# lhoyer/improving_segmentation_with_selfsupervised_depth

Measured on AMD Instinct MI355X. Metric: train images/sec, ResNet-101 joint seg+depth @512x1024, higher is better.
Workload: dtype f32

## Files before the change

### improving_segmentation_with_selfsupervised_depth_amd/csrc/winograd_fused.hip

```cpp
#include <stdlib.h>
#include <type_traits>
#include "segsde_common.h"
#include "winograd.h"
#ifndef WINO_UP_SKIP
#define WINO_UP_SKIP 1
#endif

namespace {
#define ST(s) static_cast<hipStream_t>(s)
constexpr int FT_H = 4, FT_W = 8;
constexpr int FP_H = 2 * FT_H + 2, FP_W = 2 * FT_W + 2;
constexpr int FROW = 20, FODD = FP_W / 2;
constexpr int FPS = 256;
__device__ __forceinline__ constexpr int fplane(int c) { return c * FPS + 2 * (c >> 2); }
constexpr int FCH = 64;
constexpr int FZP = 36;
constexpr int F_FLOATS = 8 * 64 * FZP > FCH * FPS ? 8 * 64 * FZP : FCH * FPS;
#ifdef WINO_DBG_OCC1
constexpr size_t F_LDS = 96 * 1024;
#else
constexpr size_t F_LDS = (size_t)F_FLOATS * sizeof(float) + 2 * 4 * 64 * sizeof(double);
#endif

struct WinoSrc { const float* x0; const float* x1; int ld0, ld1, C0, up0; };
struct WinoAg { const float* agy; int agld, agkind; };

template <bool STATS, bool UBLK, bool UPSKIP>
__global__ __launch_bounds__(256, 2) void wino_fused_kernel(WinoSrc src, int B, int H, int W, int C, int reflect,
                                                            const float* U, int ldu, int Co, const float* bias, int act, float* y, int ldy,
                                                            double* part, int accumulate, WinoAg ag) {
  SEGSDE_SMEM;
  float* lds = reinterpret_cast<float*>(segsde_smem);
  double* sh = reinterpret_cast<double*>(lds + F_FLOATS);
  const int H2 = H >> 1, W2 = W >> 1;
  const int nbw = (W2 + FT_W - 1) / FT_W, nbh = (H2 + FT_H - 1) / FT_H;
  const int tid = threadIdx.x, lane = tid & 63, wave = tid >> 6;
  const int t = lane & 31, kk = lane >> 5, th = t >> 3, tw = t & 7;
  const int bidx = blockIdx.x;
  int blk = segsde_xcd_remap(bidx, gridDim.x);
  const int bw = blk % nbw; blk /= nbw;
  const int bh = blk % nbh; const int b = blk / nbh;
  const int co0 = blockIdx.y * 64;
  const int h_top = 2 * bh * FT_H - 1, w_left = 2 * bw * FT_W - 1;
  const int a1 = wave == 0 ? 0 : (wave == 2 ? 2 : 1);
  const int a2 = wave == 0 ? 2 : (wave == 1 ? 2 : (wave == 2 ? 1 : 3));
  const float sgn = wave == 1 ? 1.f : -1.f;
  const float* pl = lds + kk * FPS + (2 * th) * FROW + tw;
  const int o1 = a1 * FROW, o2 = a2 * FROW;

  f32x16 acc[4][2];
#pragma unroll
  for (int j = 0; j < 4; ++j)
#pragma unroll
    for (int nb = 0; nb < 2; ++nb)
#pragma unroll
      for (int r = 0; r < 16; ++r) acc[j][nb][r] = 0.f;

  constexpr int NL = (FP_H * FP_W * (FCH / 4) + 255) / 256;
  unsigned poff[NL];
  int cur_src = -1, lds_ = 0;
  long img = 0;
  int sh_ = 0, Ws = 0;
  auto patch_offset = [&](int i) -> unsigned {
    const int e = tid + 256 * i;
    const int pix = e >> 4, cq = e & 15;
    const int pr = pix / FP_W, pos = pix - pr * FP_W;
    const int pc = pos < FODD ? 2 * pos : 2 * (pos - FODD) + 1;
    int hh = h_top + pr, ww = w_left + pc;
    if (reflect) {
      hh = hh < 0 ? -hh : (hh >= H ? 2 * H - 2 - hh : hh); ww = ww < 0 ? -ww : (ww >= W ? 2 * W - 2 - ww : ww);
      hh = hh < 0 ? 0 : hh; ww = ww < 0 ? 0 : ww;
    }
    const bool ok = e < FP_H * FP_W * (FCH / 4) && (unsigned)hh < (unsigned)H && (unsigned)ww < (unsigned)W;
    return ok ? (unsigned)(((hh >> sh_) * Ws + (ww >> sh_)) * lds_ + 4 * cq) * 4u : SEGSDE_OOB;
  };

  for (int c0 = 0; c0 < C; c0 += FCH) {
#ifdef WINO_DBG_LOOP_ONLY
    if (c0 == 0)
#endif
    {
    __syncthreads();
    {
      float4 v[NL];
      const int sidx = c0 < src.C0 ? 0 : 1;
      const bool first = sidx != cur_src;
      if (first) {
        cur_src = sidx;
        sh_ = (sidx == 0 && src.up0) ? 1 : 0;
        Ws = W >> sh_;
        lds_ = sidx == 0 ? src.ld0 : src.ld1;
        img = (long)(H >> sh_) * Ws * lds_;
      }
      const float* xs = sidx == 0 ? src.x0 : src.x1;
      const segsde_rsrc xr = segsde_make_rsrc(xs + (size_t)b * img + (sidx == 0 ? c0 : c0 - src.C0));
#ifdef WINO_DBG_SKIP_LOAD
      (void)xr; (void)first;
#pragma unroll
      for (int i = 0; i < NL; ++i) { poff[i] = patch_offset(i); v[i] = make_float4((float)poff[i], 1.f, 2.f, 3.f); }
#else
      if (first) {
#pragma unroll
        for (int i = 0; i < NL; ++i) { poff[i] = patch_offset(i); v[i] = segsde_buffer_load4(xr, poff[i], 0u); }
      } else {
#pragma unroll
        for (int i = 0; i < NL; ++i) v[i] = segsde_buffer_load4(xr, poff[i], 0u);
      }
#endif
#pragma unroll
      for (int i = 0; i < NL; ++i) {
        const int e = tid + 256 * i;
        if (e < FP_H * FP_W * (FCH / 4)) {
          const int pix = e >> 4, pr = pix / FP_W;
          float* d = lds + fplane(4 * (e & 15)) + pr * FROW + (pix - pr * FP_W);
          d[0] = v[i].x; d[FPS] = v[i].y; d[2 * FPS] = v[i].z; d[3 * FPS] = v[i].w;
        }
      }
    }
    __syncthreads();
    }
    const int wave_u = __builtin_amdgcn_readfirstlane(wave);
    const segsde_rsrc ur = segsde_make_rsrc(U);
    const unsigned nb64 = (unsigned)(ldu >> 6);
    const unsigned lane_off = UBLK ? (unsigned)(kk * nb64 * 256 + t * 8) * 4u : (unsigned)(kk * ldu + t) * 4u;
    const unsigned ubase = UBLK ? (unsigned)((((long)wave_u * C + c0) * nb64 + (co0 >> 6)) * 256 * 4)
                                : (unsigned)((((long)(4 * wave_u) * C + c0) * ldu + co0) * 4);
    const unsigned upos = (unsigned)((long)C * ldu * 4), ustep = UBLK ? 2u * nb64 * 256u * 4u : (unsigned)(2 * ldu * 4);
    constexpr int PD = 4, NS = FCH / 2;
    float bv[PD][8], rv[2][8];
    auto fetch_b = [&](int s, int q) {
      const unsigned so = ubase + (unsigned)s * ustep;
      if constexpr (UBLK) {
        const float4 lo = segsde_buffer_load4(ur, lane_off, so), hi = segsde_buffer_load4(ur, lane_off, so + 16u);
        bv[q][0] = lo.x; bv[q][1] = lo.y; bv[q][2] = lo.z; bv[q][3] = lo.w;
        bv[q][4] = hi.x; bv[q][5] = hi.y; bv[q][6] = hi.z; bv[q][7] = hi.w;
      } else {
#pragma unroll
        for (int j = 0; j < 4; ++j) {
          bv[q][2 * j] = segsde_buffer_load1(ur, lane_off, so + j * upos);
          bv[q][2 * j + 1] = segsde_buffer_load1(ur, lane_off, so + j * upos + 128u);
        }
      }
    };
#ifdef WINO_DBG_SKIP_K
    constexpr int NS_RUN = 1;
#else
    constexpr int NS_RUN = NS;
#endif
    float An[2][4];
    auto form_a = [&](int q, int h) {
      if (h == 0) {
        const float e0 = __builtin_fmaf(rv[0][4], sgn, rv[0][0]), e1 = __builtin_fmaf(rv[0][5], sgn, rv[0][1]);
        const float e2 = __builtin_fmaf(rv[0][6], sgn, rv[0][2]);
        An[q][0] = e0 - e2; An[q][1] = e1 + e2; An[q][2] = e2 - e1; rv[1][0] = e1;
      } else {
        const float e3 = __builtin_fmaf(rv[0][7], sgn, rv[0][3]);
        An[q][3] = rv[1][0] - e3;
      }
    };
    auto fetch_a2 = [&](int s, int bb) {
      const float* src = pl + fplane(2 * s);
      const int cp = (bb & 1) ? FODD + (bb >> 1) : (bb >> 1);
      rv[0][bb] = SEGSDE_LDS_READ_IMM(src + o1, cp); rv[0][4 + bb] = SEGSDE_LDS_READ_IMM(src + o2, cp);
    };
    const bool skip2 = UPSKIP && c0 < src.C0;
    if (!(skip2 && wave_u == 2)) {
#pragma unroll
      for (int s = 0; s < PD - 1; ++s) fetch_b(s, s);
#pragma unroll
      for (int bb = 0; bb < 4; ++bb) fetch_a2(0, bb);
      form_a(0, 0); form_a(0, 1);
      __builtin_amdgcn_sched_barrier(0);
#pragma unroll
      for (int s = 0; s < NS_RUN; ++s) {
        const int q = s & 1, qb = s % PD;
        const bool nx = s + 1 < NS;
#define WINO_MF_(j, nb, bi) acc[j][nb] = __builtin_amdgcn_mfma_f32_32x32x2f32(An[q][j], bv[qb][bi], acc[j][nb], 0, 0, 0); __builtin_amdgcn_sched_barrier(0)
        WINO_MF_(0, 0, 0); if (nx) fetch_a2(s + 1, 0); __builtin_amdgcn_sched_barrier(0);
        WINO_MF_(0, 1, 1); if (nx) fetch_a2(s + 1, 1); __builtin_amdgcn_sched_barrier(0);
        WINO_MF_(1, 0, 2); if (nx) fetch_a2(s + 1, 2); __builtin_amdgcn_sched_barrier(0);
        WINO_MF_(1, 1, 3); if (nx) fetch_a2(s + 1, 3); __builtin_amdgcn_sched_barrier(0);
        if (!skip2) {
          WINO_MF_(2, 0, 4); __builtin_amdgcn_sched_barrier(0);
          WINO_MF_(2, 1, 5); __builtin_amdgcn_sched_barrier(0);
        }
        if (s + PD - 1 < NS) fetch_b(s + PD - 1, (s + PD - 1) % PD);
        __builtin_amdgcn_sched_barrier(0);
        WINO_MF_(3, 0, 6); if (nx) form_a(q ^ 1, 0); __builtin_amdgcn_sched_barrier(0);
        WINO_MF_(3, 1, 7); if (nx) form_a(q ^ 1, 1); __builtin_amdgcn_sched_barrier(0);
#undef WINO_MF_
      }
    }
  }

#ifdef WINO_DBG_SKIP_EPI
  {
    float sdbg = 0.f;
#pragma unroll
    for (int j = 0; j < 4; ++j)
#pragma unroll
      for (int nb = 0; nb < 2; ++nb)
#pragma unroll
        for (int r = 0; r < 16; ++r) sdbg += acc[j][nb][r];
    if (sdbg == 1.2345678f) y[0] = sdbg;
    return;
  }
#endif
  __syncthreads();
  {
    float* zw = lds + ((2 * wave) * 64 + t) * FZP + 4 * kk;
#pragma unroll
    for (int nb = 0; nb < 2; ++nb)
#pragma unroll
      for (int rg = 0; rg < 4; ++rg) {
        float4 c0v, c1v;
        float* a0 = reinterpret_cast<float*>(&c0v);
        float* a1 = reinterpret_cast<float*>(&c1v);
#pragma unroll
        for (int i = 0; i < 4; ++i) {
          const int r = 4 * rg + i;
          const float m0 = acc[0][nb][r], m1 = acc[1][nb][r], m2 = acc[2][nb][r], m3 = acc[3][nb][r];
          a0[i] = (m0 + m1) + m2;
          a1[i] = (m1 - m2) - m3;
        }
        *reinterpret_cast<float4*>(zw + (nb * 32) * FZP + 8 * rg) = c0v;
        *reinterpret_cast<float4*>(zw + (64 + nb * 32) * FZP + 8 * rg) = c1v;
      }
  }
  const int n = tid & 63, tg = __builtin_amdgcn_readfirstlane(tid >> 6);
  const bool post = bias != nullptr || act != SEGSDE_ACT_NONE;
  const int co = co0 + n;
  const int ti = bh * FT_H + tg;
  const unsigned lane_b = (unsigned)co * 4u;
#ifdef WINO_EPI_POINTERS
  constexpr bool kBuf = false;
#else
  constexpr bool kBuf = true;
#endif
  const segsde_rsrc yr = segsde_make_rsrc(y + (long)b * H * W * ldy);
  const segsde_rsrc agr = segsde_make_rsrc(ag.agy ? ag.agy + (long)b * H * W * ag.agld : y);
  float agv[FT_W][4], oldv[FT_W][4];
  if (ag.agy) {
#pragma unroll
    for (int q = 0; q < FT_W; ++q) {
      const int tj = bw * FT_W + q;
      const bool ok = ti < H2 && tj < W2;
      if (kBuf) {
        const unsigned s0 = (unsigned)((2 * ti) * W + 2 * tj) * (unsigned)ag.agld * 4u, sr = (unsigned)W * (unsigned)ag.agld * 4u;
        if (ok) {
          agv[q][0] = segsde_buffer_load1(agr, lane_b, s0); agv[q][1] = segsde_buffer_load1(agr, lane_b, s0 + (unsigned)ag.agld * 4u);
          agv[q][2] = segsde_buffer_load1(agr, lane_b, s0 + sr); agv[q][3] = segsde_buffer_load1(agr, lane_b, s0 + sr + (unsigned)ag.agld * 4u);
        } else { agv[q][0] = agv[q][1] = agv[q][2] = agv[q][3] = 0.f; }
      } else {
        const float* ap = ag.agy + ((long)(b * H + 2 * ti) * W + 2 * tj) * ag.agld + co;
        agv[q][0] = ok ? ap[0] : 0.f; agv[q][1] = ok ? ap[ag.agld] : 0.f;
        agv[q][2] = ok ? ap[(long)W * ag.agld] : 0.f; agv[q][3] = ok ? ap[(long)W * ag.agld + ag.agld] : 0.f;
      }
    }
  }
  if (accumulate & 1) {
#pragma unroll
    for (int q = 0; q < FT_W; ++q) {
      const int tj = bw * FT_W + q;
      const bool ok = ti < H2 && tj < W2;
      if (kBuf) {
        const unsigned s0 = (unsigned)((2 * ti) * W + 2 * tj) * (unsigned)ldy * 4u, sr = (unsigned)W * (unsigned)ldy * 4u;
        if (ok) {
          oldv[q][0] = segsde_buffer_load1(yr, lane_b, s0); oldv[q][1] = segsde_buffer_load1(yr, lane_b, s0 + (unsigned)ldy * 4u);
          oldv[q][2] = segsde_buffer_load1(yr, lane_b, s0 + sr); oldv[q][3] = segsde_buffer_load1(yr, lane_b, s0 + sr + (unsigned)ldy * 4u);
        } else { oldv[q][0] = oldv[q][1] = oldv[q][2] = oldv[q][3] = 0.f; }
      } else {
        const float* yp = y + ((long)(b * H + 2 * ti) * W + 2 * tj) * ldy + co;
        oldv[q][0] = ok ? yp[0] : 0.f; oldv[q][1] = ok ? yp[ldy] : 0.f;
        oldv[q][2] = ok ? yp[(long)W * ldy] : 0.f; oldv[q][3] = ok ? yp[(long)W * ldy + ldy] : 0.f;
      }
    }
  }
  __syncthreads();
  const float bsv = bias ? bias[co] : 0.f;
  double ssum = 0.0, ssq = 0.0;
  float zall[4][2][FT_W];
  {
    const float* zp = lds + n * FZP + tg * FT_W;
#pragma unroll
    for (int i = 0; i < 4; ++i)
#pragma unroll
      for (int c = 0; c < 2; ++c)
#pragma unroll
        for (int h = 0; h < FT_W / 4; ++h) {
          const float4 v = *reinterpret_cast<const float4*>(zp + ((2 * i + c) * 64) * FZP + 4 * h);
          zall[i][c][4 * h] = v.x; zall[i][c][4 * h + 1] = v.y; zall[i][c][4 * h + 2] = v.z; zall[i][c][4 * h + 3] = v.w;
        }
  }
#pragma unroll
  for (int q = 0; q < FT_W; ++q) {
    float z0[4], z1[4];
#pragma unroll
    for (int i = 0; i < 4; ++i) { z0[i] = zall[i][0][q]; z1[i] = zall[i][1][q]; }
    float o[4];
    o[0] = (z0[0] + z0[1]) + z0[2]; o[1] = (z1[0] + z1[1]) + z1[2];
    o[2] = (z0[1] - z0[2]) - z0[3]; o[3] = (z1[1] - z1[2]) - z1[3];
    if (post) {
#pragma unroll
      for (int k = 0; k < 4; ++k) o[k] = segsde_act(o[k] + bsv, act);
    }
    const int tj = bw * FT_W + q;
    if (ti < H2 && tj < W2) {
      float* yp = y + ((long)(b * H + 2 * ti) * W + 2 * tj) * ldy + co;
      if (ag.agy) {
#pragma unroll
        for (int k = 0; k < 4; ++k) o[k] *= segsde_act_grad_from_out(agv[q][k], ag.agkind);
      }
      if (accumulate & 1) {
#pragma unroll
        for (int k = 0; k < 4; ++k) o[k] += oldv[q][k];
      }
#ifdef WINO_DBG_FEW_STORES
      if (q == 0)
#endif
      if (kBuf) {
        const unsigned s0 = (unsigned)((2 * ti) * W + 2 * tj) * (unsigned)ldy * 4u, sr = (unsigned)W * (unsigned)ldy * 4u, sc = (unsigned)ldy * 4u;
        if (accumulate & 2) {
          segsde_buffer_store1_nt(yr, lane_b, s0, o[0]); segsde_buffer_store1_nt(yr, lane_b, s0 + sc, o[1]);
          segsde_buffer_store1_nt(yr, lane_b, s0 + sr, o[2]); segsde_buffer_store1_nt(yr, lane_b, s0 + sr + sc, o[3]);
        } else {
          segsde_buffer_store1(yr, lane_b, s0, o[0]); segsde_buffer_store1(yr, lane_b, s0 + sc, o[1]);
          segsde_buffer_store1(yr, lane_b, s0 + sr, o[2]); segsde_buffer_store1(yr, lane_b, s0 + sr + sc, o[3]);
        }
      } else if (accumulate & 2) {
        __builtin_nontemporal_store(o[0], yp); __builtin_nontemporal_store(o[1], yp + ldy);
        __builtin_nontemporal_store(o[2], yp + (long)W * ldy); __builtin_nontemporal_store(o[3], yp + (long)W * ldy + ldy);
      } else { yp[0] = o[0]; yp[ldy] = o[1]; yp[(long)W * ldy] = o[2]; yp[(long)W * ldy + ldy] = o[3]; }
      if (STATS) {
#pragma unroll
        for (int k = 0; k < 4; ++k) { const double v = (double)o[k]; ssum += v; ssq += v * v; }
      }
    }
  }
  if (STATS) {
    sh[tg * 64 + n] = ssum; sh[256 + tg * 64 + n] = ssq;
    __syncthreads();
    if (tid < 64) {
      double a = 0.0, c2 = 0.0;
      for (int l = 0; l < 4; ++l) { a += sh[l * 64 + tid]; c2 += sh[256 + l * 64 + tid]; }
      part[((long)bidx * 2 + 0) * Co + co0 + tid] = a;
      part[((long)bidx * 2 + 1) * Co + co0 + tid] = c2;
    }
  }
}

__device__ __forceinline__ long wino_ublk_index(int r, int q, int k, int n, int K, int N) {
  return (((((long)r * K + k) * (N >> 6) + (n >> 6)) * 32 + (n & 31)) * 4 + q) * 2 + ((n >> 5) & 1);
}
__global__ __launch_bounds__(256) void wino_weight_kn_kernel(const float* w, int O, int I, int flip, float* U, int blocked) {
  const int K = flip ? O : I, N = flip ? I : O;
  const long e = blockIdx.x * 256L + threadIdx.x;
  if (e >= (long)K * N) return;
  const int nn = (int)(e % N), kq = (int)(e / N);
  const int o = flip ? kq : nn, i = flip ? nn : kq;
  const float* g = w + ((long)o * I + i) * 9;
  float k[3][3];
#pragma unroll
  for (int r = 0; r < 3; ++r)
#pragma unroll
    for (int c = 0; c < 3; ++c) k[r][c] = flip ? g[(2 - r) * 3 + (2 - c)] : g[r * 3 + c];
  float tq[4][3];
#pragma unroll
  for (int c = 0; c < 3; ++c) {
    tq[0][c] = k[0][c];
    tq[1][c] = 0.5f * ((k[0][c] + k[1][c]) + k[2][c]);
    tq[2][c] = 0.5f * ((k[0][c] - k[1][c]) + k[2][c]);
    tq[3][c] = k[2][c];
  }
  const long plane = (long)K * N;
#pragma unroll
  for (int r = 0; r < 4; ++r) {
    const float v0 = tq[r][0], v1 = 0.5f * ((tq[r][0] + tq[r][1]) + tq[r][2]), v2 = 0.5f * ((tq[r][0] - tq[r][1]) + tq[r][2]), v3 = tq[r][2];
    if (blocked) {
      float* o = U + wino_ublk_index(r, 0, kq, nn, K, N);
      o[0] = v0; o[2] = v1; o[4] = v2; o[6] = v3;
    } else {
      float* out = U + e;
      out[(4 * r + 0) * plane] = v0; out[(4 * r + 1) * plane] = v1; out[(4 * r + 2) * plane] = v2; out[(4 * r + 3) * plane] = v3;
    }
  }
}

struct BorderP {
  const float* dy; const float* wp ; float* dx; const float* agy;
  int lddy, lddx, agld, agkind, B, H, W, Cin, Cout, mode, nseg, ldw;
};

__global__ __launch_bounds__(256) void reflect_borders_kernel(BorderP p) {
  SEGSDE_SMEM;
  float* sh = reinterpret_cast<float*>(segsde_smem);
  const int tid = threadIdx.x, lane = tid & 63, wave = tid >> 6, m = lane & 31, kk = lane >> 5;
  const int L = p.mode == 0 ? p.W : p.H;
  int r = blockIdx.x;
  const int seg = r % p.nseg; r /= p.nseg;
  const int far = r & 1, b = r >> 1;
  const int p0 = seg * 32, pitch = p.Cout + 1, cq4 = p.Cout >> 2;
  const int fixed = p.mode == 0 ? (far ? p.H - 1 : 0) : (far ? p.W - 1 : 0);
  for (int idx = tid; idx < 34 * cq4; idx += 256) {
    const int px = idx / cq4, q = idx - px * cq4, pos = p0 - 1 + px;
    float4 v = make_float4(0.f, 0.f, 0.f, 0.f);
    if (pos >= 0 && pos < L) {
      const long pix = p.mode == 0 ? ((long)(b * p.H + fixed) * p.W + pos) : ((long)(b * p.H + pos) * p.W + fixed);
      v = *reinterpret_cast<const float4*>(p.dy + pix * p.lddy + 4 * q);
    }
    float* d = sh + px * pitch + 4 * q;
    d[0] = v.x; d[1] = v.y; d[2] = v.z; d[3] = v.w;
  }
  __syncthreads();
  const int ktap = far ? 2 : 0;
  const bool top = p.mode == 1 && p0 <= 1 && 1 < p0 + 32, bot = p.mode == 1 && p0 <= p.H - 2 && p.H - 2 < p0 + 32;
  const int steps = p.Cout >> 1;
  for (int nb = wave; nb < (p.Cin >> 5); nb += 4) {
    const int cin = nb * 32 + m;
    f32x16 acc;
#pragma unroll
    for (int q = 0; q < 16; ++q) acc[q] = 0.f;
    for (int t = 0; t < 5; ++t) {
      if (t == 3 && !top) continue;
      if (t == 4 && !bot) continue;
      int kh, kw, src; bool mine = true;
      if (t < 3) {
        kh = p.mode == 0 ? ktap : t; kw = p.mode == 0 ? t : ktap; src = m + 2 - t;
      } else {
        kh = t == 3 ? 0 : 2; kw = ktap;
        const int at = t == 3 ? 1 : p.H - 2;
        mine = p0 + m == at;
        src = (t == 3 ? 0 : p.H - 1) - (p0 - 1);
      }
      const float* ap = sh + src * pitch + kk;
      const float* bp = p.wp + ((long)kk * 9 + kh * 3 + kw) * p.ldw + cin;
      const long bstep = 18L * p.ldw;
      float bv[2][8];
#pragma unroll
      for (int u = 0; u < 8; ++u) bv[0][u] = u < steps ? bp[u * bstep] : 0.f;
      for (int s0 = 0; s0 < steps; s0 += 16) {
#pragma unroll
        for (int half = 0; half < 2; ++half) {
          const int sb = s0 + 8 * half;
          if (sb < steps) {
#pragma unroll
            for (int u = 0; u < 8; ++u) bv[half ^ 1][u] = sb + 8 + u < steps ? bp[(long)(sb + 8 + u) * bstep] : 0.f;
#pragma unroll
            for (int u = 0; u < 8; ++u) {
              if (sb + u < steps) {
                const float a = mine ? ap[2 * (sb + u)] : 0.f;
                acc = __builtin_amdgcn_mfma_f32_32x32x2f32(a, bv[half][u], acc, 0, 0, 0);
              }
            }
          }
        }
      }
    }
#pragma unroll
    for (int q = 0; q < 16; ++q) {
      const int row = (q & 3) + 8 * (q >> 2) + 4 * kk, pos = p0 + row;
      if (pos < L) {
        const long pix = p.mode == 0 ? ((long)(b * p.H + (far ? p.H - 2 : 1)) * p.W + pos) : ((long)(b * p.H + pos) * p.W + (far ? p.W - 2 : 1));
        float v = acc[q];
        if (p.agy) v *= segsde_act_grad_from_out(p.agy[pix * p.agld + cin], p.agkind);
        p.dx[pix * p.lddx + cin] += v;
      }
    }
  }
}

}
int segsde_wino_ublk() {
  static int v = -1;
  if (v < 0) { const char* e = getenv("SEGSDE_WINO_FUSED_UBLK"); v = e ? (atoi(e) != 0) : 1; }
  return v;
}
namespace {
inline long fused_blocks(int B, int H, int W) {
  return (long)B * (((H >> 1) + FT_H - 1) / FT_H) * (((W >> 1) + FT_W - 1) / FT_W);
}
}

extern "C" int segsde_winograd_fused_ok(int B, int H, int W, int C, int Cout) {
  return B > 0 && H >= 4 && W >= 4 && H % 2 == 0 && W % 2 == 0 && C >= FCH && C % FCH == 0 && Cout >= 64 && Cout % 64 == 0 &&
         (long)H * W * (C > Cout ? C : Cout) * 4 < (1L << 31) &&
         fused_blocks(B, H, W) < (1L << 31) && (long)B * H * W * (C > Cout ? C : Cout) < (1L << 40);
}

extern "C" long segsde_winograd_fused_stats_rows(int B, int H, int W) { return fused_blocks(B, H, W); }

extern "C" int segsde_winograd_fused_pack(const float* w_oihw, int O, int I, int flip, float* U, void* stream) {
  if (!w_oihw || !U) return SEGSDE_ERR_NULL;
  if (O <= 0 || I <= 0) return SEGSDE_ERR_SHAPE;
  const long total = (long)O * I;
  const int blocked = segsde_wino_ublk() && ((flip ? I : O) % 64 == 0);
  hipLaunchKernelGGL(wino_weight_kn_kernel, dim3((unsigned)((total + 255) / 256)), dim3(256), 0, ST(stream), w_oihw, O, I, flip, U, blocked);
  SEGSDE_CHECK_LAUNCH();
  return 0;
}

namespace {
int launch_fused(const WinoSrc& src, int B, int H, int W, int C, int reflect, const float* u_kn, int ldu, int Cout, const float* bias, int act,
                 float* y, int ldy, int accumulate, double* stats, const WinoAg& ag, void* stream) {
  const dim3 grid((unsigned)fused_blocks(B, H, W), (unsigned)(Cout / 64));
  const bool ublk = segsde_wino_ublk() != 0;
  static long nt_bytes = -1;
  if (nt_bytes < 0) { const char* e = getenv("SEGSDE_WINO_NT_MB"); nt_bytes = (e ? atol(e) : 200L) << 20; }
  accumulate = (accumulate ? 1 : 0) | ((nt_bytes > 0 && (long)B * H * W * Cout * 4 >= nt_bytes) ? 2 : 0);
  auto go = [&](auto k, double* st) {
    (void)hipFuncSetAttribute(reinterpret_cast<const void*>(k), hipFuncAttributeMaxDynamicSharedMemorySize, (int)F_LDS);
    hipLaunchKernelGGL(k, grid, dim3(256), F_LDS, ST(stream), src, B, H, W, C, reflect, u_kn, ldu, Cout, bias, act, y, ldy, st, accumulate, ag);
  };
  static int upskip_on = -1;
  if (upskip_on < 0) { const char* e = getenv("SEGSDE_WINO_UP_SKIP"); upskip_on = e ? (atoi(e) != 0) : 1; }
  const bool upskip = WINO_UP_SKIP && upskip_on && src.up0;
  auto pick = [&](auto st_tag, double* st) {
    constexpr bool ST = decltype(st_tag)::value;
    if (upskip) { if (ublk) go(wino_fused_kernel<ST, true, true>, st); else go(wino_fused_kernel<ST, false, true>, st); }
    else { if (ublk) go(wino_fused_kernel<ST, true, false>, st); else go(wino_fused_kernel<ST, false, false>, st); }
  };
  if (stats) pick(std::true_type{}, stats); else pick(std::false_type{}, (double*)nullptr);
  SEGSDE_CHECK_LAUNCH();
  return 0;
}
inline bool pitch_ok(int H, int W, int ld) { return (long)H * W * ld * 4 < (1L << 31); }
}

extern "C" int segsde_conv2d_winograd_fused(const float* x, int ldx, int B, int H, int W, int C, int reflect, const float* u_kn,
                                            int Cout, const float* bias, int act, float* y, int ldy, int accumulate, double* stats,
                                            void* stream) {
  if (!x || !u_kn || !y) return SEGSDE_ERR_NULL;
  if (!segsde_winograd_fused_ok(B, H, W, C, Cout) || ldx < C || ldx % 4 != 0 || !pitch_ok(H, W, ldx) || ldy < Cout || !pitch_ok(H, W, ldy) || (accumulate && (stats || bias || act)))
    return SEGSDE_ERR_UNSUPPORTED;
  const WinoSrc src{x, nullptr, ldx, 0, C, 0};
  return launch_fused(src, B, H, W, C, reflect, u_kn, Cout, Cout, bias, act, y, ldy, accumulate, stats, WinoAg{nullptr, 0, 0}, stream);
}

extern "C" int segsde_conv2d_winograd_fused2(const float* x0, int ld0, int C0, int up0, const float* x1, int ld1, int C1, int B, int H,
                                             int W, int reflect, const float* u_kn, int Cout, const float* bias, int act, float* y,
                                             int ldy, double* stats, void* stream) {
  if (!x0 || !u_kn || !y || (C1 > 0 && !x1)) return SEGSDE_ERR_NULL;
  const int C = C0 + (C1 > 0 ? C1 : 0);
  if (!segsde_winograd_fused_ok(B, H, W, C, Cout) || C0 <= 0 || C0 % FCH || ld0 < C0 || ld0 % 4 != 0 || (C1 > 0 && (ld1 < C1 || ld1 % 4 != 0 || !pitch_ok(H, W, ld1))) ||
      !pitch_ok(H >> (up0 ? 1 : 0), W >> (up0 ? 1 : 0), ld0) || ldy < Cout || !pitch_ok(H, W, ldy))
    return SEGSDE_ERR_UNSUPPORTED;
  const WinoSrc src{x0, x1, ld0, ld1, C0, up0 ? 1 : 0};
  return launch_fused(src, B, H, W, C, reflect, u_kn, Cout, Cout, bias, act, y, ldy, 0, stats, WinoAg{nullptr, 0, 0}, stream);
}

extern "C" int segsde_conv2d_winograd_fused_dgrad(const float* dy, int lddy, int B, int H, int W, int Cout, const float* ud_kn, int ldu,
                                                  int Cin, float* dx, int lddx, int accumulate, const float* act_out, int act_ld,
                                                  int act_kind, void* stream) {
  if (!dy || !ud_kn || !dx) return SEGSDE_ERR_NULL;
  if (!segsde_winograd_fused_ok(B, H, W, Cout, Cin) || ldu < Cin || (long)16 * Cout * ldu >= (1L << 28) || lddy < Cout || lddy % 4 != 0 || !pitch_ok(H, W, lddy) || lddx < Cin || !pitch_ok(H, W, lddx) ||
      (act_out && (act_kind < SEGSDE_ACT_RELU || act_kind > SEGSDE_ACT_SIGMOID || act_ld < Cin || !pitch_ok(H, W, act_ld))))
    return SEGSDE_ERR_UNSUPPORTED;
  const WinoSrc src{dy, nullptr, lddy, 0, Cout, 0};
  return launch_fused(src, B, H, W, Cout, 0, ud_kn, ldu, Cin, nullptr, SEGSDE_ACT_NONE, dx, lddx, accumulate, nullptr,
                      WinoAg{act_out, act_ld, act_kind}, stream);
}

extern "C" int segsde_reflect_adjoint_borders2(const float* dy, int lddy, const float* wpack, int ldw, float* dx, int lddx,
                                               const float* act_out, int act_ld, int act_kind, int B, int H, int W, int Cin, int Cout,
                                               void* stream) {
  if (!dy || !wpack || !dx) return SEGSDE_ERR_NULL;
  if (B <= 0 || H < 4 || W < 4 || Cin <= 0 || Cin % 32 || ldw < Cin || Cout <= 0 || Cout % 32 || Cout > 1024 || lddy < Cout || lddy % 4 || lddx < Cin ||
      ((uintptr_t)dy & 15) || (act_out && (act_kind < SEGSDE_ACT_RELU || act_kind > SEGSDE_ACT_SIGMOID || act_ld < Cin)))
    return SEGSDE_ERR_UNSUPPORTED;
  BorderP p;
  p.dy = dy; p.wp = wpack; p.dx = dx; p.agy = act_out; p.lddy = lddy; p.lddx = lddx; p.agld = act_ld; p.agkind = act_kind;
  p.B = B; p.H = H; p.W = W; p.Cin = Cin; p.Cout = Cout; p.ldw = ldw;
  const size_t lb = (size_t)34 * (Cout + 1) * sizeof(float);
  (void)hipFuncSetAttribute(reinterpret_cast<const void*>(reflect_borders_kernel), hipFuncAttributeMaxDynamicSharedMemorySize, (int)lb);
  for (int mode = 0; mode < 2; ++mode) {
    p.mode = mode; p.nseg = ((mode == 0 ? W : H) + 31) / 32;
    hipLaunchKernelGGL(reflect_borders_kernel, dim3((unsigned)(B * 2 * p.nseg)), dim3(256), lb, ST(stream), p);
    SEGSDE_CHECK_LAUNCH();
  }
  return 0;
}
```

Before: 64.52.

## Split reflect-border adjoint across Cin blocks and software-pipeline weight loads

The border adjoint kernel now launches a second grid dimension over input-channel blocks, so each wave handles one 32-channel block instead of looping over all of them. Weight loads are triple-buffered in groups of 16 across taps and steps, and the dx/activation reads are issued before the shared-memory staging of dy. The dy staging loop is batched to issue several float4 loads before storing. This adds parallelism and hides load latency, but each Cin block now stages the same dy border strip redundantly and uses more registers.

```diff
diff --git a/improving_segmentation_with_selfsupervised_depth_amd/csrc/winograd_fused.hip b/improving_segmentation_with_selfsupervised_depth_amd/csrc/winograd_fused.hip
--- a/improving_segmentation_with_selfsupervised_depth_amd/csrc/winograd_fused.hip
+++ b/improving_segmentation_with_selfsupervised_depth_amd/csrc/winograd_fused.hip
@@ -390,6 +390,8 @@
   const float* dy; const float* wp ; float* dx; const float* agy;
   int lddy, lddx, agld, agkind, B, H, W, Cin, Cout, mode, nseg, ldw;
 };
+constexpr int BORDER_WG = 16;
+constexpr int BORDER_SB = 9;
 
 __global__ __launch_bounds__(256) void reflect_borders_kernel(BorderP p) {
   SEGSDE_SMEM;
@@ -400,71 +402,110 @@
   const int seg = r % p.nseg; r /= p.nseg;
   const int far = r & 1, b = r >> 1;
   const int p0 = seg * 32, pitch = p.Cout + 1, cq4 = p.Cout >> 2;
+  const int nb = blockIdx.y * 4 + wave;
+  const bool active = nb < (p.Cin >> 5);
+  const int cin = nb * 32 + m;
   const int fixed = p.mode == 0 ? (far ? p.H - 1 : 0) : (far ? p.W - 1 : 0);
-  for (int idx = tid; idx < 34 * cq4; idx += 256) {
-    const int px = idx / cq4, q = idx - px * cq4, pos = p0 - 1 + px;
-    float4 v = make_float4(0.f, 0.f, 0.f, 0.f);
-    if (pos >= 0 && pos < L) {
-      const long pix = p.mode == 0 ? ((long)(b * p.H + fixed) * p.W + pos) : ((long)(b * p.H + pos) * p.W + fixed);
-      v = *reinterpret_cast<const float4*>(p.dy + pix * p.lddy + 4 * q);
-    }
-    float* d = sh + px * pitch + 4 * q;
-    d[0] = v.x; d[1] = v.y; d[2] = v.z; d[3] = v.w;
-  }
-  __syncthreads();
   const int ktap = far ? 2 : 0;
   const bool top = p.mode == 1 && p0 <= 1 && 1 < p0 + 32, bot = p.mode == 1 && p0 <= p.H - 2 && p.H - 2 < p0 + 32;
   const int steps = p.Cout >> 1;
-  for (int nb = wave; nb < (p.Cin >> 5); nb += 4) {
-    const int cin = nb * 32 + m;
-    f32x16 acc;
-#pragma unroll
-    for (int q = 0; q < 16; ++q) acc[q] = 0.f;
-    for (int t = 0; t < 5; ++t) {
-      if (t == 3 && !top) continue;
-      if (t == 4 && !bot) continue;
-      int kh, kw, src; bool mine = true;
-      if (t < 3) {
-        kh = p.mode == 0 ? ktap : t; kw = p.mode == 0 ? t : ktap; src = m + 2 - t;
-      } else {
-        kh = t == 3 ? 0 : 2; kw = ktap;
-        const int at = t == 3 ? 1 : p.H - 2;
-        mine = p0 + m == at;
-        src = (t == 3 ? 0 : p.H - 1) - (p0 - 1);
-      }
-      const float* ap = sh + src * pitch + kk;
-      const float* bp = p.wp + ((long)kk * 9 + kh * 3 + kw) * p.ldw + cin;
-      const long bstep = 18L * p.ldw;
-      float bv[2][8];
-#pragma unroll
-      for (int u = 0; u < 8; ++u) bv[0][u] = u < steps ? bp[u * bstep] : 0.f;
-      for (int s0 = 0; s0 < steps; s0 += 16) {
-#pragma unroll
-        for (int half = 0; half < 2; ++half) {
-          const int sb = s0 + 8 * half;
-          if (sb < steps) {
-#pragma unroll
-            for (int u = 0; u < 8; ++u) bv[half ^ 1][u] = sb + 8 + u < steps ? bp[(long)(sb + 8 + u) * bstep] : 0.f;
-#pragma unroll
-            for (int u = 0; u < 8; ++u) {
-              if (sb + u < steps) {
-                const float a = mine ? ap[2 * (sb + u)] : 0.f;
-                acc = __builtin_amdgcn_mfma_f32_32x32x2f32(a, bv[half][u], acc, 0, 0, 0);
-              }
-            }
-          }
-        }
-      }
-    }
-#pragma unroll
-    for (int q = 0; q < 16; ++q) {
-      const int row = (q & 3) + 8 * (q >> 2) + 4 * kk, pos = p0 + row;
-      if (pos < L) {
-        const long pix = p.mode == 0 ? ((long)(b * p.H + (far ? p.H - 2 : 1)) * p.W + pos) : ((long)(b * p.H + pos) * p.W + (far ? p.W - 2 : 1));
-        float v = acc[q];
-        if (p.agy) v *= segsde_act_grad_from_out(p.agy[pix * p.agld + cin], p.agkind);
-        p.dx[pix * p.lddx + cin] += v;
-      }
+  const long wstep = 18L * p.ldw;
+  struct Cursor { int t, s0; };
+  auto advance = [&](Cursor& c) {
+    c.s0 += BORDER_WG;
+    if (c.s0 >= steps) {
+      c.s0 = 0; ++c.t;
+      if (c.t == 3 && !top) ++c.t;
+      if (c.t == 4 && !bot) ++c.t;
+    }
+  };
+  auto wload = [&](float (&bv)[BORDER_WG], const Cursor& c) {
+    const int t = c.t < 5 ? c.t : 0;
+    const int kh = t < 3 ? (p.mode == 0 ? ktap : t) : (t == 3 ? 0 : 2), kw = t < 3 ? (p.mode == 0 ? t : ktap) : ktap;
+    const float* bp = p.wp + ((long)kk * 9 + kh * 3 + kw) * p.ldw + cin + c.s0 * wstep;
+#pragma unroll
+    for (int u = 0; u < BORDER_WG; ++u) bv[u] = bp[u * wstep];
+  };
+  float bv0[BORDER_WG], bv1[BORDER_WG], bv2[BORDER_WG];
+  Cursor wl{0, 0};
+  if (active) {
+    wload(bv0, wl); advance(wl);
+    wload(bv1, wl); advance(wl);
+  }
+  const long pix0 = p.mode == 0 ? ((long)(b * p.H + (far ? p.H - 2 : 1)) * p.W + p0) : ((long)(b * p.H + p0) * p.W + (far ? p.W - 2 : 1));
+  const long pstride = p.mode == 0 ? 1 : p.W;
+  float dxv[16], agv[16];
+#pragma unroll
+  for (int q = 0; q < 16; ++q) {
+    const int row = (q & 3) + 8 * (q >> 2) + 4 * kk;
+    const long pix = pix0 + row * pstride;
+    const bool ok = active && p0 + row < L;
+    dxv[q] = ok ? p.dx[pix * p.lddx + cin] : 0.f;
+    agv[q] = (ok && p.agy) ? p.agy[pix * p.agld + cin] : 0.f;
+  }
+  {
+    int px = tid / cq4, q = tid - px * cq4;
+    const int dpx = 256 / cq4, dq = 256 - dpx * cq4, total = 34 * cq4;
+    for (int i0 = tid; i0 < total; i0 += 256 * BORDER_SB) {
+      float4 v[BORDER_SB];
+      int pxs = px, qs = q;
+#pragma unroll
+      for (int j = 0; j < BORDER_SB; ++j) {
+        const int pos = p0 - 1 + px;
+        v[j] = make_float4(0.f, 0.f, 0.f, 0.f);
+        if (i0 + 256 * j < total && pos >= 0 && pos < L) {
+          const long pix = p.mode == 0 ? ((long)(b * p.H + fixed) * p.W + pos) : ((long)(b * p.H + pos) * p.W + fixed);
+          v[j] = *reinterpret_cast<const float4*>(p.dy + pix * p.lddy + 4 * q);
+        }
+        px += dpx; q += dq;
+        if (q >= cq4) { q -= cq4; ++px; }
+      }
+#pragma unroll
+      for (int j = 0; j < BORDER_SB; ++j) {
+        if (i0 + 256 * j < total) {
+          float* d = sh + pxs * pitch + 4 * qs;
+          d[0] = v[j].x; d[1] = v[j].y; d[2] = v[j].z; d[3] = v[j].w;
+        }
+        pxs += dpx; qs += dq;
+        if (qs >= cq4) { qs -= cq4; ++pxs; }
+      }
+    }
+  }
+  __syncthreads();
+  if (!active) return;
+  f32x16 acc;
+#pragma unroll
+  for (int q = 0; q < 16; ++q) acc[q] = 0.f;
+  Cursor c{0, 0};
+  auto group = [&](const float (&cur)[BORDER_WG], float (&nxt)[BORDER_WG]) {
+    wload(nxt, wl); advance(wl);
+    bool mine = true;
+    int src = m + 2 - c.t;
+    if (c.t >= 3) {
+      const int at = c.t == 3 ? 1 : p.H - 2;
+      mine = p0 + m == at;
+      src = (c.t == 3 ? 0 : p.H - 1) - (p0 - 1);
+    }
+    const float* ap = sh + src * pitch + kk + 2 * c.s0;
+    float a[BORDER_WG];
+#pragma unroll
+    for (int u = 0; u < BORDER_WG; ++u) a[u] = ap[2 * u];
+#pragma unroll
+    for (int u = 0; u < BORDER_WG; ++u) acc = __builtin_amdgcn_mfma_f32_32x32x2f32(mine ? a[u] : 0.f, cur[u], acc, 0, 0, 0);
+    advance(c);
+  };
+  while (true) {
+    group(bv0, bv2); if (c.t >= 5) break;
+    group(bv1, bv0); if (c.t >= 5) break;
+    group(bv2, bv1); if (c.t >= 5) break;
+  }
+#pragma unroll
+  for (int q = 0; q < 16; ++q) {
+    const int row = (q & 3) + 8 * (q >> 2) + 4 * kk;
+    if (p0 + row < L) {
+      float v = acc[q];
+      if (p.agy) v *= segsde_act_grad_from_out(agv[q], p.agkind);
+      p.dx[(pix0 + row * pstride) * p.lddx + cin] = dxv[q] + v;
     }
   }
 }
@@ -574,7 +615,7 @@
   (void)hipFuncSetAttribute(reinterpret_cast<const void*>(reflect_borders_kernel), hipFuncAttributeMaxDynamicSharedMemorySize, (int)lb);
   for (int mode = 0; mode < 2; ++mode) {
     p.mode = mode; p.nseg = ((mode == 0 ? W : H) + 31) / 32;
-    hipLaunchKernelGGL(reflect_borders_kernel, dim3((unsigned)(B * 2 * p.nseg)), dim3(256), lb, ST(stream), p);
+    hipLaunchKernelGGL(reflect_borders_kernel, dim3((unsigned)(B * 2 * p.nseg), (unsigned)((Cin + 127) / 128)), dim3(256), lb, ST(stream), p);
     SEGSDE_CHECK_LAUNCH();
   }
   return 0;
```

After: 64.80, median of 6. About the same (+0.4%).
